# metagentools/VStrains

Measured on AMD Instinct MI355X. Metric: PE read pairs/sec through PE-link inference (GFA index + packed reads in HBM -> node_mat/short_mat), higher is better.
Workload: dtype u32

## Files before the change

### vstrains_amd/csrc/vs_api.hip

```cpp
#include <stdarg.h>
#include <stdio.h>
#include <stdlib.h>
#include <string.h>

#include "vs_internal.h"

static thread_local std::string g_create_err;

int vs_fail(vs_ctx *ctx, int code, const char *fmt, ...) {
    char buf[512];
    va_list ap;
    va_start(ap, fmt);
    vsnprintf(buf, sizeof buf, fmt, ap);
    va_end(ap);
    if (ctx) ctx->err = buf; else g_create_err = buf;
    return code;
}

static bool env_on(const char *name) {
    const char *v = getenv(name);
    return v && atoi(v) != 0;
}

void vs_tuning_load(VsTuning &t, bool experiment) {
    t = VsTuning();
    if (!experiment) return;
    if (const char *v = getenv("VS_EPT")) t.ept = (uint32_t)atoi(v) & ~1u;
    if (const char *v = getenv("VS_GRID_PER_CU")) t.grid_per_cu = atoi(v) > 0 ? (uint32_t)atoi(v) : 128u;
    if (const char *v = getenv("VS_ACC_FILL")) t.acc_fill_pct = atoi(v);
    if (const char *v = getenv("VS_ACC_TASKS")) t.acc_tasks = atoi(v) > 0 ? (uint32_t)atoi(v) : 0u;
    if (const char *v = getenv("VS_SHORTCUT")) t.shortcut = atoi(v) != 0 ? 1 : 0;
    if (const char *v = getenv("VS_ADAPT_GRID")) t.adapt_grid = atoi(v) != 0 ? 1 : 0;
    if (const char *v = getenv("VS_ACC_ROWS")) t.acc_rows = atoi(v) != 0 ? 1 : 0;
    if (const char *v = getenv("VS_LTAB_BITS")) t.ltab_bits = atoi(v) >= 0 && atoi(v) <= 31 ? atoi(v) : -1;
    if (const char *v = getenv("VS_ROWS_KEYS")) t.rows_keys = atoi(v) >= 2 && atoi(v) <= 65536 ? (uint32_t)atoi(v) : 0u;
    if (const char *v = getenv("VS_ROWS_SUB")) t.rows_sub = atoi(v) >= 1024 ? (uint32_t)atoi(v) : 0u;
    if (const char *v = getenv("VS_ROWS_PER_STRIP")) t.rows_per_strip = atoi(v) > 0 && atoi(v) <= 64 ? (uint32_t)atoi(v) : 0u;
    if (const char *v = getenv("VS_LOCUS_STAGE")) t.locus_stage = atoi(v) >= 0 ? atoi(v) : -1;
    t.no_sort = env_on("VS_NO_SORT");
    t.locus_global = env_on("VS_LOCUS_GLOBAL");
    t.no_fast = env_on("VS_NO_FAST");
    t.no_std = env_on("VS_NO_STD");
    t.no_agg = env_on("VS_NO_AGG");
    t.no_mid = env_on("VS_NO_MID");
}

extern "C" {

int vs_abi_version(void) { return VS_ABI_VERSION; }

int vs_device_count(void) {
    int n = 0;
    if (hipGetDeviceCount(&n) != hipSuccess) return 0;
    return n;
}

const char *vs_last_error(const vs_ctx *ctx) { return ctx ? ctx->err.c_str() : g_create_err.c_str(); }

int vs_ctx_create(int device, vs_ctx **out) {
    if (!out) return vs_fail(nullptr, VS_E_ARG, "vs_ctx_create: out is NULL");
    *out = nullptr;
    int n = 0;
    hipError_t e = hipGetDeviceCount(&n);
    if (e != hipSuccess || n <= 0)
        return vs_fail(nullptr, VS_E_HIP, "no HIP device available (%s); this library has no CPU path",
                       e == hipSuccess ? "device count 0" : hipGetErrorString(e));
    if (device < 0 || device >= n) return vs_fail(nullptr, VS_E_ARG, "device %d out of range (0..%d)", device, n - 1);
    e = hipSetDevice(device);
    if (e != hipSuccess) return vs_fail(nullptr, VS_E_HIP, "hipSetDevice(%d): %s", device, hipGetErrorString(e));
    vs_ctx *ctx = new vs_ctx();
    ctx->device = device;
    if (const char *ev = getenv("VS_EXPERIMENT")) ctx->experiment = strcmp(ev, "1") == 0;
    vs_tuning_load(ctx->tune, ctx->experiment);
    hipDeviceProp_t prop;
    if (hipGetDeviceProperties(&prop, device) == hipSuccess) ctx->n_cu = prop.multiProcessorCount;
    for (int i = 0; i < 5; i++) {
        e = hipEventCreate(&ctx->ev[i]);
        if (e != hipSuccess) {
            int rc = vs_fail(nullptr, VS_E_HIP, "hipEventCreate: %s", hipGetErrorString(e));
            delete ctx;
            return rc;
        }
    }
    *out = ctx;
    return VS_OK;
}

static void free_index(vs_ctx *ctx) {
    ctx->d_meta.reset();
    ctx->d_fwd.reset();
    ctx->d_table.reset();
    ctx->d_post.reset();
    ctx->d_slot_node.reset();
    ctx->has_index = false;
    ctx->index_bytes = 0;
}

void vs_ctx_free_index(vs_ctx *ctx) { free_index(ctx); }

void vs_ctx_destroy(vs_ctx *ctx) {
    if (!ctx) return;
    (void)hipSetDevice(ctx->device);
    (void)hipStreamSynchronize(ctx->stream);
    for (FqStage &st : ctx->fq_stage) {
        if (st.in_flight && st.done) (void)hipEventSynchronize(st.done);
        if (st.done) (void)hipEventDestroy(st.done);
    }
    for (int i = 0; i < 5; i++)
        if (ctx->ev[i]) (void)hipEventDestroy(ctx->ev[i]);
    delete ctx;
}

int vs_ctx_set_stream(vs_ctx *ctx, void *stream) {
    if (!ctx) return VS_E_ARG;
    ctx->stream = (hipStream_t)stream;
    return VS_OK;
}

int vs_ctx_keep_masks(vs_ctx *ctx, int on) {
    if (!ctx) return VS_E_ARG;
    ctx->keep_masks = on != 0;
// ... 170 lines not shown
```

### vstrains_amd/csrc/vs_pe.hip

```cpp
#include <stdio.h>
#include <stdlib.h>
#include <string.h>

#include <vector>

#include "vs_internal.h"
#include "vs_acc_tasks.h"
#include "vs_pe_pack.h"

#define TPB 256
#define LCAP 20u
__device__ __forceinline__ const uint32_t *vs_row_quad(const uint32_t *__restrict__ lists, const uint32_t *__restrict__ hi, uint64_t row, uint32_t q) {
    return q < LC / 4u ? lists + row * LC + 4u * q : hi + row * 4u;
}
#define EMPTY_NODE 0xFFFFFFFFu

struct PeParams {
    VsIndexDev idx;
    VsReadsDev rd;
    uint32_t *node_mat, *short_mat;
    unsigned long long *stats;
    uint32_t ept, pmax, words_cap, pool, pool_bits;
    uint64_t n_tiles;
    uint32_t *slow_list, *slow_count;
// ... 1502 lines not shown
                    const uint32_t ys[4] = {yv.x, yv.y, yv.z, yv.w};
                    uint32_t key[4], seen[4], at[4];
#pragma unroll
                    for (uint32_t j = 0; j < 4u; j++) {
                        key[j] = kbase + ys[j];
                        at[j] = RsTable::slot(key[j]);
                        seen[j] = s_key[at[j]];
                    }
#pragma unroll
                    for (uint32_t j = 0; j < 4u; j++) {
                        if (q4 + j >= n || (MODE && ys[j] < x)) continue;
                        if (seen[j] == key[j]) {
                            atomicAdd(&s_cnt[at[j]], wgt);
                        } else if (!vs_cell_claim<RsTable>(s_key, s_cnt, &s_used, key[j], at[j], wgt)) {
                            atomicAdd(&s_lost, 1u);
                            vs_mark_tile(tile_map, T, (uint32_t)MODE, x, ys[j]);
                            atomicAdd(mat + cell0 + (key[j] - align), wgt);
                        }
                    }
                };
                add_quad(yq, 4u * q);
                if (n > 16u && q == 0u) add_quad(*(const VsQuad *)(lists_hi + (uint64_t)(p0 & 0x07FFFFFFu) * 4u), 16u);
            }
            if ((pass & 3u) == 3u) {
                __syncthreads();
                const bool spill = s_used > fill_limit || s_lost > 4096u;
                __syncthreads();
                if (spill) write_out();
            }
        }
        __syncthreads();
        write_out();
    }
}

#define VS_LOCUS_MISS 0xFFFFFFFFu
__device__ __forceinline__ uint32_t vs_locus_probe(const VsIndexDev &idx, uint64_t key) {
    const uint32_t mask = (1u << idx.table_bits) - 1u;
    uint32_t sl = vs_slot_of(key, idx.table_bits);
    const uint4 *tab = (const uint4 *)idx.table;
    for (;;) {
        const uint4 raw = tab[sl];
        const uint32_t node = idx.slot_node[sl];
        const uint64_t k = (uint64_t)raw.x | ((uint64_t)raw.y << 32);
        if (k == VS_EMPTY_KEY) return VS_LOCUS_MISS;
        if ((k & ~VS_MULTI_BIT) == key) return node;
        sl = (sl + 1u) & mask;
    }
}

__device__ __forceinline__ uint32_t vs_locus_key(const VsIndexDev &idx, const VsReadsDev &rd, uint64_t p) {
    const uint32_t mf = rd.meta[2 * p], mr = rd.meta[2 * p + 1];
    const uint32_t N = idx.n_nodes, w = idx.w, s = idx.s, K = idx.K;
    if ((((mf | mr) >> 24) & VS_FLAG_N) || (mf & VS_LEN_MASK) < K || (mr & VS_FILTER_LEN_MASK) < K) return N + 1u;
    const uint32_t rlen = mf & VS_LEN_MASK;
    const uint64_t base = (uint64_t)rd.woff[2 * p] * 16u;
    const bool inv = (mf >> 24) & VS_FLAG_INVALID;
    for (uint32_t j = vs_seed_phase(rlen, w, s); j + w <= rlen; j += s) {
        if (inv && vs_seed_dirty(rd.mask, base + j, w)) continue;
        uint32_t sr;
        const uint64_t key = vs_seed_key(rd.words, base + j, w, &sr);
        const uint32_t node = vs_locus_probe(idx, key);
        if (node != VS_LOCUS_MISS) return node;
    }
    return N;
}

__device__ __forceinline__ uint32_t vs_locus_key_end(const VsIndexDev &idx, const VsReadsDev &rd, uint64_t e) {
    const uint32_t m = rd.meta[e];
    const uint32_t N = idx.n_nodes, w = idx.w, s = idx.s, rlen = m & VS_LEN_MASK;
    const uint64_t base = (uint64_t)rd.woff[e] * 16u;
    const bool inv = (m >> 24) & VS_FLAG_INVALID;
    for (uint32_t j = vs_seed_phase(rlen, w, s); j + w <= rlen; j += s) {
        if (inv && vs_seed_dirty(rd.mask, base + j, w)) continue;
        uint32_t sr;
        const uint64_t key = vs_seed_key(rd.words, base + j, w, &sr);
        const uint32_t node = vs_locus_probe(idx, key);
        if (node != VS_LOCUS_MISS) return node;
    }
    return N;
}

#define LOCUS_TPB 1024
__global__ void __launch_bounds__(LOCUS_TPB)
k_locus_count(VsIndexDev idx, VsReadsDev rd, uint64_t n_pairs, uint32_t chunk, uint32_t n_wg, uint32_t *__restrict__ keys,
              uint32_t *__restrict__ cnt, uint32_t key_lo, uint32_t nk, uint32_t compute) {
    for (uint32_t i = threadIdx.x; i < nk; i += LOCUS_TPB) vs_lds[i] = 0;
    __syncthreads();
    const uint64_t lo = (uint64_t)blockIdx.x * chunk;
    const uint64_t hi = lo + chunk < n_pairs ? lo + chunk : n_pairs;
    for (uint64_t p = lo + threadIdx.x; p < hi; p += LOCUS_TPB) {
        uint32_t key;
        if (compute) {
            key = vs_locus_key(idx, rd, p);
            keys[p] = key;
        } else {
            key = keys[p];
        }
        if (key - key_lo < nk) atomicAdd(&vs_lds[key - key_lo], 1u);
    }
    __syncthreads();
    for (uint32_t i = threadIdx.x; i < nk; i += LOCUS_TPB) cnt[(uint64_t)(key_lo + i) * n_wg + blockIdx.x] = vs_lds[i];
}

struct LocusHdr {
    uint32_t mf, mr, ws, we, w0;
    bool live;
};
typedef uint32_t LocusQuad __attribute__((ext_vector_type(4)));
struct LocusQuads {
    LocusQuad q0, q1, q2, q3, q4;
};
struct LocusProbe {
    uint32_t res, j, sl, node, rlen, lbase;
    uint64_t key, gbase;
    uint4 raw;
    bool have, active, inv;
};
__global__ void __launch_bounds__(LOCUS_TPB)
k_locus_count_staged(VsIndexDev idx, VsReadsDev rd, uint64_t n_pairs, uint32_t chunk, uint32_t n_wg, uint32_t *__restrict__ keys,
                     uint32_t *__restrict__ cnt, uint32_t nk, uint32_t cap) {
    static_assert(LOCUS_STAGE_PAIRS == 64u && LOCUS_TPB / 64u == LOCUS_STAGE_WAVES, "a batch holds one pair per lane of a wavefront");
    const uint32_t tid = threadIdx.x, lane = tid & 63u, wv = tid >> 6;
    const uint32_t hist_words = (nk + 3u) & ~3u, buf_words = vs_locus_buf_words(cap);
    uint32_t *s_hist = vs_lds;
    uint32_t *s_buf = vs_lds + hist_words + wv * 2u * buf_words;
    for (uint32_t i = tid; i < nk; i += LOCUS_TPB) s_hist[i] = 0;
    __syncthreads();
    const uint64_t c_lo = (uint64_t)blockIdx.x * chunk, c_hi = c_lo + chunk < n_pairs ? c_lo + chunk : n_pairs;
    const uint32_t sub = (chunk + LOCUS_STAGE_WAVES - 1u) / LOCUS_STAGE_WAVES;
    const uint64_t hi = c_lo + (uint64_t)(wv + 1u) * sub < c_hi ? c_lo + (uint64_t)(wv + 1u) * sub : c_hi;
    const uint64_t lo = c_lo + (uint64_t)wv * sub < hi ? c_lo + (uint64_t)wv * sub : hi;
    const bool any = lo < hi;
    const uint32_t N = idx.n_nodes, w = idx.w, s = idx.s, K = idx.K, tmask = (1u << idx.table_bits) - 1u;
    const uint4 *tab = (const uint4 *)idx.table;

    auto load_hdr = [&](uint64_t P) -> LocusHdr {
        LocusHdr h = {0u, 0u, 0u, 0u, 0u, false};
        if (!any) return h;
        const uint64_t Pc = P < hi ? P : hi - 1u, q = P + lane < hi ? P + lane : hi - 1u;
        const uint2 m = *(const uint2 *)(rd.meta + 2u * q);
        h.mf = m.x;
        h.mr = m.y;
        h.ws = rd.woff[2u * q];
        h.we = rd.woff[2u * q + 2u];
        h.w0 = rd.woff[2u * Pc];
        h.live = P + lane < hi;
        return h;
    };
    auto cut = [&](const LocusHdr &h, uint32_t &w_end) -> uint32_t {
        const uint64_t m = __ballot(vs_locus_in_batch(h.live, h.w0, h.we, cap));
        const uint32_t n = (uint32_t)__popcll(m);
        w_end = n ? (uint32_t)__shfl((int)h.we, (int)(n - 1u)) : 0u;
        return n;
    };
#define LOCUS_EACH_QUAD(X) X(0) X(1) X(2) X(3) X(4)
    static_assert(LOCUS_STAGE_QUADS == 5u, "LOCUS_EACH_QUAD names the quads");
    auto stage_load = [&](bool on, uint32_t w_first, uint32_t w_end, LocusQuads &r) {
        LocusSpan sp = vs_locus_span(on ? w_first : 0u, on ? w_end : 0u);
        if (sp.quads > buf_words / 4u) sp.quads = buf_words / 4u;
        const LocusQuad *src = (const LocusQuad *)(rd.words + sp.first);
#define LOCUS_LOAD(k) r.q##k = src[lane + k * 64u < sp.quads ? lane + k * 64u : sp.quads - 1u];
        LOCUS_EACH_QUAD(LOCUS_LOAD)
#undef LOCUS_LOAD
    };
    auto stage_store = [&](bool on, uint32_t w_first, uint32_t w_end, const LocusQuads &r, uint32_t *buf) {
// ... 24 lines not shown
            return;
        }
        if (k == VS_EMPTY_KEY) {
            q.j += s;
            q.active = seek(q);
        } else {
            q.sl = (q.sl + 1u) & tmask;
        }
        if (q.active) {
            q.raw = tab[q.sl];
            q.node = idx.slot_node[q.sl];
        }
    };
    auto finish = [&](const LocusProbe &q, uint64_t p_first) {
        if (q.have) {
            keys[p_first + lane] = q.res;
            if (q.res < nk) atomicAdd(&s_hist[q.res], 1u);
        }
    };

    LocusQuads r;
    uint64_t pc = lo, po = lo;
    LocusHdr hc = load_hdr(pc);
    uint32_t wec, wen;
    uint32_t nc = cut(hc, wec);
    bool stc = nc != 0u;
    if (!nc && pc < hi) nc = 1u;
    stage_load(stc, hc.w0, wec, r);
    stage_store(stc, hc.w0, wec, r, s_buf);
    uint64_t pn = pc + nc;
    LocusHdr hn = load_hdr(pn);
    uint32_t nn = cut(hn, wen);
    bool stn = nn != 0u;
    if (!nn && pn < hi) nn = 1u;
    LocusProbe qo = {};
    for (uint32_t it = 0; pc < hi; it++) {
        LocusProbe qc = {};
        qc.have = lane < nc;
        qc.res = N + 1u;
        qc.rlen = hc.mf & VS_LEN_MASK;
        qc.inv = (hc.mf >> 24) & VS_FLAG_INVALID;
        qc.lbase = ((it & 1u) * buf_words + hc.ws - (hc.w0 & ~3u)) * 16u;
        qc.gbase = (uint64_t)hc.ws * 16u;
        if (qc.have && !stc) {
            qc.res = vs_locus_key(idx, rd, pc);
        } else if (qc.have && !((((hc.mf | hc.mr) >> 24) & VS_FLAG_N) || qc.rlen < K || (hc.mr & VS_FILTER_LEN_MASK) < K)) {
            qc.res = N;
            qc.j = vs_seed_phase(qc.rlen, w, s);
            qc.active = seek(qc);
        }
        if (!qc.active) qc.sl = 0;
        qc.raw = tab[qc.sl];
        qc.node = idx.slot_node[qc.sl];
        stage_load(stn, hn.w0, wen, r);
        const uint64_t p2 = pn + nn;
        const LocusHdr h2 = load_hdr(p2);
        look(qo);
        look(qc);
        while (qo.active) {
            look(qo);
            look(qc);
        }
        finish(qo, po);
        stage_store(stn, hn.w0, wen, r, s_buf + ((it + 1u) & 1u) * buf_words);
        uint32_t we2;
        uint32_t n2 = cut(h2, we2);
        const bool st2 = n2 != 0u;
        if (!n2 && p2 < hi) n2 = 1u;
        qo.res = qc.res; qo.j = qc.j; qo.sl = qc.sl; qo.node = qc.node; qo.rlen = qc.rlen; qo.lbase = qc.lbase; qo.key = qc.key;
        qo.gbase = qc.gbase; qo.raw = qc.raw; qo.have = qc.have; qo.active = qc.active; qo.inv = qc.inv;
        po = pc;
        pc = pn; hc = hn; nc = nn; stc = stn; wec = wen;
        pn = p2; hn = h2; nn = n2; stn = st2; wen = we2;
    }
    while (qo.active) look(qo);
    finish(qo, po);
    __syncthreads();
    for (uint32_t i = tid; i < nk; i += LOCUS_TPB) cnt[(uint64_t)i * n_wg + blockIdx.x] = s_hist[i];
}

__global__ void __launch_bounds__(LOCUS_TPB)
k_locus_scatter(uint32_t key_lo, uint32_t nk, uint64_t n_pairs, uint32_t chunk, uint32_t n_wg, const uint32_t *__restrict__ keys,
                const uint32_t *__restrict__ first, uint32_t *__restrict__ perm) {
    for (uint32_t i = threadIdx.x; i < nk; i += LOCUS_TPB) vs_lds[i] = first[(uint64_t)(key_lo + i) * n_wg + blockIdx.x];
    __syncthreads();
    const uint64_t lo = (uint64_t)blockIdx.x * chunk;
    const uint64_t hi = lo + chunk < n_pairs ? lo + chunk : n_pairs;
    for (uint64_t p = lo + threadIdx.x; p < hi; p += LOCUS_TPB) {
        const uint32_t key = keys[p];
        if (key - key_lo < nk) perm[atomicAdd(&vs_lds[key - key_lo], 1u)] = (uint32_t)p;
    }
}

__global__ void __launch_bounds__(TPB)
k_pe_locus(VsIndexDev idx, VsReadsDev rd, uint64_t n_pairs, uint32_t *__restrict__ keys, uint32_t *__restrict__ hist) {
    const uint64_t p = (uint64_t)blockIdx.x * TPB + threadIdx.x;
    if (p >= n_pairs) return;
    const uint32_t key = vs_locus_key(idx, rd, p);
    keys[p] = key;
    atomicAdd(&hist[key], 1u);
}

__global__ void __launch_bounds__(TPB)
k_pe_permute(uint64_t n_pairs, const uint32_t *__restrict__ keys, uint32_t *__restrict__ cursor, uint32_t *__restrict__ perm) {
    const uint64_t p = (uint64_t)blockIdx.x * TPB + threadIdx.x;
    if (p >= n_pairs) return;
    perm[atomicAdd(&cursor[keys[p]], 1u)] = (uint32_t)p;
}

#define MID_SLOTS 256u
#define MID_LIST 64u
#define MID_WORDS (4u * MID_SLOTS + 3u * 64u + 65u + 2u * MID_LIST + 4u)
__global__ void __launch_bounds__(TPB)
k_pe_mid(PeParams P, const uint32_t *__restrict__ in_list, const uint32_t *__restrict__ in_count, uint32_t in_cap,
         uint32_t *__restrict__ out_list, uint32_t *__restrict__ out_count) {
    __shared__ uint32_t s_all[(TPB / 64u) * MID_WORDS];
    const uint32_t lane = threadIdx.x & 63u, wv = threadIdx.x >> 6;
    uint32_t *s_key = s_all + wv * MID_WORDS, *s_cnt = s_key + MID_SLOTS, *s_minp = s_cnt + MID_SLOTS, *s_minj = s_minp + MID_SLOTS;
    uint32_t *s_pa = s_minj + MID_SLOTS, *s_pb = s_pa + 64u, *s_pc = s_pb + 64u, *s_pref = s_pc + 64u;
    uint32_t *s_lst = s_pref + 65u;
    uint32_t *s_flag = s_lst + 2u * MID_LIST;
    const uint32_t N = P.idx.n_nodes, w = P.idx.w, s = P.idx.s, K = P.idx.K, wv_seed = VS_SEED_VERIFIED(P.idx.w);
    uint32_t n_in = *in_count;
    if (n_in > in_cap) n_in = in_cap;
    const uint32_t n_waves = gridDim.x * (TPB / 64u);
    for (uint32_t li = blockIdx.x * (TPB / 64u) + wv; li < n_in; li += n_waves) {
        const uint32_t pair = in_list[li];
        if (lane < 4u) s_flag[lane] = 0u;
        vs_wave_sync();
        for (uint32_t side = 0; side < 2u; side++) {
            const uint64_t e = 2ull * pair + side;
            const uint32_t meta = P.rd.meta[e];
            const uint32_t rlen = meta & VS_LEN_MASK;
            const uint64_t rbase = (uint64_t)P.rd.woff[e] * 16u;
            const uint32_t *mk = ((meta >> 24) & VS_FLAG_INVALID) ? P.rd.mask : nullptr;
            const uint32_t nprobe = vs_seed_probes(rlen, w, s), phase = vs_seed_phase(rlen, w, s);
            for (uint32_t i = lane; i < MID_SLOTS; i += 64u) { s_key[i] = EMPTY_NODE; s_cnt[i] = 0u; s_minp[i] = 0xFFFFFFFFu; s_minj[i] = 0xFFFFFFFFu; }
            if (nprobe > 64u) { if (lane == 0u) s_flag[0] = 1u; }
            uint32_t c = 0u, pa = 0u, pb = 0u;
            if (lane < nprobe && nprobe <= 64u) {
                const uint32_t j = phase + lane * s;
                if (!(mk && vs_seed_dirty(mk, rbase + j, w))) {
                    uint32_t sr;
                    const uint64_t key = vs_seed_key(P.rd.words, rbase + j, w, &sr);
                    c = vs_probe(P.idx, key, sr, &pa, &pb);
                }
            }
            uint32_t incl = c;
#pragma unroll
            for (int d = 1; d < 64; d <<= 1) {
                const uint32_t t2 = __shfl_up(incl, d, 64);
                if (lane >= (uint32_t)d) incl += t2;
            }
            s_pa[lane] = pa; s_pb[lane] = pb; s_pc[lane] = c;
            s_pref[lane + 1u] = incl;
            if (lane == 0u) s_pref[0] = 0u;
            vs_wave_sync();
            const uint32_t total = s_pref[64];
            for (uint32_t t = lane; t < total; t += 64u) {
                const uint32_t pr = vs_upper_idx(s_pref, 65u, t);
                const uint32_t k2 = t - s_pref[pr], j = phase + pr * s;
                uint32_t node, pos, opp;
                VsNodeMeta nm;
                if (s_pc[pr] == 1u) {
                    node = s_pa[pr]; pos = s_pb[pr] & 0x7FFFFFFFu; opp = s_pb[pr] >> 31;
                    nm = P.idx.meta[node];
                } else {
                    const VsPosting po = vs_posting_unpack(P.idx.postings[s_pa[pr] + k2]);
                    node = po.node; pos = po.pos; opp = po.strand ^ (s_pb[pr] >> 31);
                    nm.woff = po.woff; nm.len = po.len;
                }
                const uint32_t q = opp ? nm.len - pos - w : pos;
                uint32_t a, qa, len;
// ... 382 lines not shown
    VS_HIP(ctx, ctx->d_dense.reserve(pl.dense_bytes, pl.dense_bytes, &dense_new));
    if (dense_new) {
        ctx->dense_nodes = idx.n_nodes;
        uint64_t N = idx.n_nodes ? idx.n_nodes : 1;
        VS_HIP(ctx, hipMemsetAsync(ctx->d_dense.ptr(), 0xFF, pl.dense_bytes, st));
        hipLaunchKernelGGL(k_dense_zero_cnt, dim3((unsigned)((N * pl.slow_grid + TPB - 1) / TPB)), dim3(TPB), 0, st,
                           ctx->d_dense.as<uint32_t>(), N, (uint64_t)pl.slow_grid);
    }
    VS_HIP(ctx, hipMemsetAsync(ctx->d_slow_count.ptr(), 0, sizeof(uint32_t) * vs_ctx::SC_WORDS, st));
    if (pl.use_sort) {
        VS_HIP(ctx, ctx->d_locus_keys.reserve(sizeof(uint32_t) * n_pairs));
        VS_HIP(ctx, ctx->d_perm.reserve(sizeof(uint32_t) * n_pairs));
        VS_HIP(ctx, ctx->d_locus_hist.reserve(sizeof(uint32_t) * pl.locus_hist_words));
        VS_HIP(ctx, ctx->d_scan_tmp.reserve(sizeof(uint64_t) * (pl.locus_hist_words / 2048 + 4)));
    }
    if (d_node_mat) {
        VS_HIP(ctx, ctx->d_lists.reserve(sizeof(uint32_t) * pl.list_words));
        VS_HIP(ctx, ctx->d_list_counts.reserve(sizeof(uint32_t) * (pl.list_ends + 2)));
    }

    PeParams P;
    P.idx = idx;
    P.rd = reads->dev();
    P.out_lists = ctx->d_lists.as<uint32_t>();
    P.out_counts = ctx->d_list_counts.as<uint32_t>();
    P.node_mat = d_node_mat;
    P.short_mat = d_short_mat;
    P.stats = (unsigned long long *)d_stats;
    P.ept = pl.ept;
    P.pmax = pl.pmax;
    P.words_cap = pl.words_cap;
    P.pool = pl.pool;
    P.pool_bits = pl.pool_bits;
    P.n_pairs = n_pairs;
    P.n_tiles = pl.n_tiles;
    P.tiles_per_wg = pl.tiles_per_wg;
    P.wpe = pl.wpe;
    P.magic_pmax = pl.magic_pmax;
    P.magic_wpe = pl.magic_wpe;
    P.perm = pl.use_sort ? ctx->d_perm.as<const uint32_t>() : nullptr;
    P.slow_list = ctx->d_slow_list.as<uint32_t>();
    P.slow_count = ctx->d_slow_count.as<uint32_t>();
    P.dbg_lists = d_dbg_lists;
    P.dbg_counts = d_dbg_counts;
    P.dbg_cap = dbg_cap;
    P.accumulate = d_node_mat ? 1u : 0u;
    P.out_rows = pl.use_rows;
    P.out_lists_hi = ctx->d_lists.as<uint32_t>() + pl.list_ends * LC;
    P.tile_map = d_node_mat ? d_tile_map : nullptr;
    P.tile_T = (idx.n_nodes + 63u) >> 6;
    P.shortcut = pl.shortcut;
    P.mid_fast = pl.mid_fast;

    const size_t lds = pl.lds_bytes;
    if (lds > 64u * 1024u)
        VS_HIP(ctx, hipFuncSetAttribute(tf->fn, hipFuncAttributeMaxDynamicSharedMemorySize, (int)lds));
    VS_HIP(ctx, hipEventRecord(ctx->ev[3], st));
    ctx->last_order_pairs = n_pairs;
    if (pl.use_sort) {
        const uint64_t nk = pl.locus_keys;
        ctx->last_launched |= pl.lds_sort ? VS_RAN_LOCUS_LDS_SORT : VS_RAN_LOCUS_GLOBAL_SORT;
        if (pl.lds_sort) {
            const uint32_t n_wg = LOCUS_WGS, chunk = pl.locus_chunk, per_pass = pl.locus_per_pass;
            const size_t lds_keys = sizeof(uint32_t) * per_pass;
            if (lds_keys > 64u * 1024u) {
                VS_HIP(ctx, hipFuncSetAttribute((const void *)k_locus_count, hipFuncAttributeMaxDynamicSharedMemorySize, (int)lds_keys));
                VS_HIP(ctx, hipFuncSetAttribute((const void *)k_locus_scatter, hipFuncAttributeMaxDynamicSharedMemorySize, (int)lds_keys));
            }
            if (pl.locus_stage_words && ((uintptr_t)reads->d_words & 15u) == 0u) {
                VS_HIP(ctx, hipFuncSetAttribute((const void *)k_locus_count_staged, hipFuncAttributeMaxDynamicSharedMemorySize, (int)pl.locus_lds_bytes));
                hipLaunchKernelGGL(k_locus_count_staged, dim3(n_wg), dim3(LOCUS_TPB), pl.locus_lds_bytes, st, idx, reads->dev(), n_pairs, chunk, n_wg,
                                   ctx->d_locus_keys.as<uint32_t>(), ctx->d_locus_hist.as<uint32_t>(), (uint32_t)nk, pl.locus_stage_words);
                ctx->last_launched |= VS_RAN_LOCUS_STAGED;
            } else {
                for (uint32_t key_lo = 0; key_lo < nk; key_lo += per_pass) {
                    const uint32_t n_here = (uint32_t)(nk - key_lo < per_pass ? nk - key_lo : per_pass);
                    hipLaunchKernelGGL(k_locus_count, dim3(n_wg), dim3(LOCUS_TPB), lds_keys, st, idx, reads->dev(), n_pairs, chunk, n_wg,
                                       ctx->d_locus_keys.as<uint32_t>(), ctx->d_locus_hist.as<uint32_t>(), key_lo, n_here, key_lo == 0u ? 1u : 0u);
                }
            }
            int rc = vs_scan_u32(ctx, ctx->d_locus_hist.as<const uint32_t>(), ctx->d_locus_hist.as<uint32_t>(), nk * n_wg,
                                 ctx->d_scan_tmp.as<uint64_t>(), nullptr);
            if (rc) return rc;
            for (uint32_t key_lo = 0; key_lo < nk; key_lo += per_pass) {
                const uint32_t n_here = (uint32_t)(nk - key_lo < per_pass ? nk - key_lo : per_pass);
                hipLaunchKernelGGL(k_locus_scatter, dim3(n_wg), dim3(LOCUS_TPB), lds_keys, st, key_lo, n_here, n_pairs, chunk, n_wg,
                                   ctx->d_locus_keys.as<const uint32_t>(), ctx->d_locus_hist.as<const uint32_t>(), ctx->d_perm.as<uint32_t>());
            }
        } else {
            VS_HIP(ctx, hipMemsetAsync(ctx->d_locus_hist.ptr(), 0, sizeof(uint32_t) * nk, st));
            const unsigned pg = (unsigned)((n_pairs + TPB - 1) / TPB);
            hipLaunchKernelGGL(k_pe_locus, dim3(pg), dim3(TPB), 0, st, idx, reads->dev(), n_pairs, ctx->d_locus_keys.as<uint32_t>(),
                               ctx->d_locus_hist.as<uint32_t>());
            int rc = vs_scan_u32(ctx, ctx->d_locus_hist.as<const uint32_t>(), ctx->d_locus_hist.as<uint32_t>(), nk,
                                 ctx->d_scan_tmp.as<uint64_t>(), nullptr);
            if (rc) return rc;
            hipLaunchKernelGGL(k_pe_permute, dim3(pg), dim3(TPB), 0, st, n_pairs, ctx->d_locus_keys.as<const uint32_t>(),
                               ctx->d_locus_hist.as<uint32_t>(), ctx->d_perm.as<uint32_t>());
        }
    }
    VS_HIP(ctx, hipEventRecord(ctx->ev[0], st));
    if (!d_node_mat) VS_HIP(ctx, hipEventRecord(ctx->ev[4], st));
    ctx->last_kernel = tf->name;
    {
        void *kargs[] = {(void *)&P};
        VS_HIP(ctx, hipLaunchKernel(tf->fn, dim3((unsigned)pl.grid), dim3(TTPB), kargs, lds, st));
    }
    if (d_node_mat) {
        const StdTable tab = pl.sw ? vs_std_table((int)pl.mode, true, pl.ad != 0u) : StdTable{pl.pool, 0u};
        ctx->last_handoff.pairs = n_pairs;
        ctx->last_handoff.list_ends = pl.list_ends;
        ctx->last_handoff.ept = pl.ept;
        ctx->last_handoff.rows = pl.use_rows;
        ctx->last_handoff.pool = tab.pool;
        ctx->last_handoff.trim = tab.trim;
        const int rc = pe_count_from_lists(ctx, pl, idx.n_nodes, 2ull * n_pairs, d_node_mat, d_short_mat, d_tile_map);
        if (rc) return rc;
    }
    VS_HIP(ctx, hipEventRecord(ctx->ev[1], st));
    const bool no_mid = ctx->tune.no_mid;
    ctx->last_launched |= no_mid ? 0u : VS_RAN_PE_MID;
    if (!no_mid) {
        hipLaunchKernelGGL(k_pe_mid, dim3((unsigned)ctx->n_cu * 8u), dim3(TPB), 0, st, P, ctx->d_slow_list.as<const uint32_t>(),
                           ctx->d_slow_count.as<const uint32_t>(), (uint32_t)n_pairs, ctx->d_slow_list2.as<uint32_t>(), ctx->d_slow_count.as<uint32_t>() + vs_ctx::SC_SLOW);
        hipLaunchKernelGGL(k_pe_slow, dim3(pl.slow_grid), dim3(TPB), 0, st, P, ctx->d_dense.as<uint32_t>(), (uint32_t)n_pairs,
                           ctx->d_slow_list2.as<const uint32_t>(), ctx->d_slow_count.as<const uint32_t>() + vs_ctx::SC_SLOW);
    } else {
        hipLaunchKernelGGL(k_pe_slow, dim3(pl.slow_grid), dim3(TPB), 0, st, P, ctx->d_dense.as<uint32_t>(), (uint32_t)n_pairs,
                           ctx->d_slow_list.as<const uint32_t>(), ctx->d_slow_count.as<const uint32_t>());
    }
    ctx->last_overflow.pairs = n_pairs;
    ctx->last_overflow.no_mid = no_mid ? 1u : 0u;
    VS_HIP(ctx, hipEventRecord(ctx->ev[2], st));
    VS_HIP(ctx, hipGetLastError());
    return VS_OK;
}

extern "C" int vs_pe_count(vs_ctx *ctx, const vs_reads *reads, uint32_t *d_node_mat, uint32_t *d_short_mat, uint64_t *d_stats) {
    if (!ctx || !reads || !d_node_mat || !d_short_mat || !d_stats) return VS_E_ARG;
    return pe_launch(ctx, reads, d_node_mat, d_short_mat, d_stats, nullptr, nullptr, 0);
}

extern "C" int vs_pe_count_tracked(vs_ctx *ctx, const vs_reads *reads, uint32_t *d_node_mat, uint32_t *d_short_mat, uint64_t *d_stats,
                                   uint8_t *d_tile_map) {
    if (!ctx || !reads || !d_node_mat || !d_short_mat || !d_stats || !d_tile_map) return VS_E_ARG;
    return pe_launch(ctx, reads, d_node_mat, d_short_mat, d_stats, nullptr, nullptr, 0, d_tile_map);
}

extern "C" int vs_counts_zero_tracked(vs_ctx *ctx, uint32_t *d_node_mat, uint32_t *d_short_mat, uint32_t n, uint8_t *d_tile_map) {
    if (!ctx || (n && (!d_node_mat || !d_short_mat || !d_tile_map))) return vs_fail(ctx, VS_E_ARG, "vs_counts_zero_tracked: bad argument");
    if (!n) return VS_OK;
    VS_HIP(ctx, hipSetDevice(ctx->device));
    const uint32_t T = (n + 63u) >> 6;
    const uint64_t tiles = 2ull * T * T;
    if (tiles > 0x7FFFFFFFull) return vs_fail(ctx, VS_E_RANGE, "vs_counts_zero_tracked: %u nodes make more tiles than one launch takes", n);
    hipLaunchKernelGGL(k_zero_tiles, dim3((unsigned)((tiles + 63u) / 64u)), dim3(64), 0, ctx->stream, d_node_mat, d_short_mat, n, T, d_tile_map, tiles);
    VS_HIP(ctx, hipGetLastError());
    return VS_OK;
}

static PePlan pe_lists_plan(vs_ctx *ctx, uint32_t n_nodes, uint64_t n_ends, bool tile_map) {
    if (ctx->experiment) vs_tuning_load(ctx->tune, true);
    PePlanIn in;
    in.n_nodes = n_nodes; in.K = STD_K; in.w = STD_W; in.s = STD_S;
    in.n_cu = (uint32_t)ctx->n_cu;
    in.n_ends = n_ends; in.max_len = 150u;
    in.count = true; in.tile_map = tile_map;
    in.tune = ctx->tune;
// ... 303 lines not shown
```

### vstrains_amd/csrc/vs_pe_plan.h

```cpp
#ifndef VS_PE_PLAN_H
#define VS_PE_PLAN_H
#include <stddef.h>
#include <stdint.h>
#include <stdio.h>

#include <initializer_list>

#include "../../include/vstrains_hip.h"

#if defined(__HIPCC__)
#define VS_PLAN_FN __host__ __device__ inline
#else
#define VS_PLAN_FN inline
#endif

struct VsTuning {
    uint32_t ept = 0;
    uint32_t grid_per_cu = 128;
    int acc_fill_pct = -1;
    uint32_t acc_tasks = 0;
    int shortcut = -1;
    int adapt_grid = -1;
    int acc_rows = -1;
    int ltab_bits = -1;
    uint32_t rows_keys = 0, rows_sub = 0;
    uint32_t rows_per_strip = 0;
    bool no_sort = false, locus_global = false, no_fast = false, no_std = false, no_agg = false;
    bool no_mid = false;
    int locus_stage = -1;
};

VS_PLAN_FN uint32_t vs_seed_phase(uint32_t len, uint32_t w, uint32_t s) {
    return len < w ? 0u : ((len - w) % s + s) / 2u;
}
VS_PLAN_FN uint32_t vs_seed_probes(uint32_t len, uint32_t w, uint32_t s) {
    if (len < w) return 0u;
    return (len - w + 1u) / s;
}
#define VS_SEED_VERIFIED(w) ((w) <= 31u ? (w) : 0u)

#define LC 16u
#define PPT 2u
#define TTPB 256
#define PPT_LONG 1u
#define CHUNK (TTPB * PPT)
#define ACC_TPB 1024
#define ACC_BITS 14
#define ACC_SLOTS (1u << ACC_BITS)
#define ACC_PPW 64u
#define ACC_TASK_WORDS 480u
#define ACC_TASK_CAP (2u * ACC_TASK_WORDS)
#define ACC_TASK_MIN 40u
#define ACC_QUEUE 64u
#define ACC_TASK_PLAN_CAP (ACC_TASK_CAP - 2u * ACC_QUEUE)
#define ACC_BINS 24u
#define ROWS_KEYS 65536u
#define ROWS_SUB ((1u << 26) - 1024u)
#define RS_BITS 13
#define RS_SLOTS (1u << RS_BITS)
#define LOCUS_LDS_KEYS 36864u
#define LOCUS_LDS_MAX_PASSES 4u
#define LOCUS_WGS 256u
#define LOCUS_STAGE_WAVES 16u
#define LOCUS_STAGE_PAIRS 64u
#define LOCUS_STAGE_QUADS 5u
#define LOCUS_STAGE_SLACK 16u
#define LOCUS_STAGE_MAX (LOCUS_STAGE_QUADS * 4u * LOCUS_STAGE_PAIRS - LOCUS_STAGE_SLACK)
#define LOCUS_STAGE_MIN_PAIRS 48u
#define LOCUS_LDS_WORDS 40960u
#define SLOW_WORDS_PER_NODE 6u
#define LDS_BUDGET_BYTES (64u * 1024u)
#define NI_CAP 4096u

VS_PLAN_FN bool vs_locus_in_batch(bool exists, uint32_t w_first, uint32_t w_pair_end, uint32_t cap) {
    return exists && w_pair_end - w_first <= cap;
}
struct LocusBatch {
    uint32_t n;
    uint32_t staged;
};
VS_PLAN_FN LocusBatch vs_locus_batch(const uint32_t *woff, uint64_t p0, uint64_t hi, uint32_t cap) {
    LocusBatch b = {0u, 1u};
    if (p0 >= hi) return b;
    const uint32_t w_first = woff[2u * p0];
    while (b.n < LOCUS_STAGE_PAIRS && vs_locus_in_batch(p0 + b.n < hi, w_first, p0 + b.n < hi ? woff[2u * (p0 + b.n) + 2u] : 0u, cap)) b.n++;
    if (!b.n) { b.n = 1u; b.staged = 0u; }
    return b;
}
struct LocusSpan {
    uint32_t first, quads;
};
VS_PLAN_FN LocusSpan vs_locus_span(uint32_t w_first, uint32_t w_end) {
    LocusSpan sp;
    sp.first = w_first & ~3u;
    sp.quads = (w_end + 4u - sp.first + 3u) / 4u;
    return sp;
}
VS_PLAN_FN uint32_t vs_locus_buf_words(uint32_t cap) { return ((cap + 3u) & ~3u) + LOCUS_STAGE_SLACK; }

struct TileLayout {
    uint32_t woff, gend, meta, inv, words, pcnt, pa, pb, hkey, hcnt, hminp, hminj, ns, state, list, owner, misc, total;
};
VS_PLAN_FN TileLayout tile_layout(uint32_t ept, uint32_t pmax, uint32_t words_cap, uint32_t pool, uint32_t list_trim = 0u) {
    TileLayout t;
    uint32_t o = 0;
    const uint32_t NI = ept * pmax;
    t.woff = o;  o += 2u * ((ept + 2u) & ~1u);
    t.gend = o;  o += 2u * ept;
    t.meta = o;  o += 2u * ept;
    t.inv = o;   o += ept;
    t.words = o; o += 2u * (words_cap + 8u);
    t.pcnt = o;  o += NI + 1u;
    t.pa = o;    o += NI;
    t.pb = o;    o += NI;
    t.hkey = o;  o += pool;
    t.hcnt = o;  o += pool;
    t.hminp = o; o += pool;
    t.hminj = o; o += pool;
    t.ns = o;    o += ept;
    t.state = o; o += ept;
    t.list = o;
    t.owner = o; o += (ept * LC - list_trim > CHUNK ? ept * LC - list_trim : CHUNK);
    t.misc = o;  o += 16u;
    t.total = o;
    return t;
}

#define STD_EPT (TTPB / 4u)
#define STD_POOL_BITS 10u
#define STD_K 56u
#define STD_W 31u
#define STD_S 26u
#define STD2_EPT 60u
#define STD2_POOL_BITS 10u
#define STD2_K 128u
#define STD2_W 63u
#define STD2_S 66u
struct StdShape {
    uint32_t mode, sw, sp;
};
constexpr StdShape VS_STD_SHAPES[] = {{1u, 10u, 4u}, {1u, 8u, 3u}, {1u, 7u, 2u}, {1u, 7u, 3u}, {2u, 16u, 2u}};
struct StdTable {
    uint32_t pool, trim;
};
VS_PLAN_FN constexpr StdTable vs_std_table(int mode, bool std_shape, bool ad) {
    return std_shape && !ad ? StdTable{768u, mode == 2 ? 192u : 64u} : StdTable{1u << (mode == 2 ? STD2_POOL_BITS : STD_POOL_BITS), 0u};
}

inline uint32_t slow_grid_for(uint32_t n_nodes) {
    const uint64_t per_wg = sizeof(uint32_t) * (uint64_t)SLOW_WORDS_PER_NODE * (n_nodes ? n_nodes : 1u);
    uint64_t g = (4ull << 30) / per_wg;
    return (uint32_t)(g < 64u ? 64u : g > 2048u ? 2048u : g);
}

inline uint32_t pool_for(uint32_t ept, uint32_t *bits) {
    uint32_t b = 6;
    while ((1u << b) < 16u * ept) b++;
    *bits = b;
    return 1u << b;
}

inline size_t lds_bytes(uint32_t ept, uint32_t pmax, uint32_t words_cap) {
    uint32_t bits;
    uint32_t pool = pool_for(ept, &bits);
    return (size_t)tile_layout(ept, pmax, words_cap, pool).total * sizeof(uint32_t);
}

struct PePlanIn {
    uint32_t n_nodes = 0, K = 0, w = 0, s = 0;
    uint64_t n_seed_pos = 0, n_distinct = 0;
    uint32_t max_node_len = 0, n_cu = 0;
    uint64_t n_ends = 0;
    uint32_t max_len = 0;
    bool has_mask = false, has_inv4 = false;
    bool count = false, tile_map = false;
    VsTuning tune;
};

struct PePlan {
    int status;
    char msg[128];
    uint32_t ept, pmax, wpe, pool, pool_bits, words_cap, magic_pmax, magic_wpe;
    uint64_t lds_bytes;
    uint32_t mode, sw, sp, ad;
    uint64_t n_tiles, grid, list_ends, list_words;
    uint32_t tiles_per_wg, shortcut, mid_fast;
    uint32_t use_sort, lds_sort, locus_chunk, locus_per_pass;
    uint64_t locus_keys, locus_hist_words;
    uint32_t locus_stage_words;
    uint64_t locus_lds_bytes;
    uint32_t use_rows, use_table, mark_tiles;
    uint32_t acc_grid, acc_per_wg, acc_fill, acc_task_cap;
    uint64_t rows_sub_pairs;
    uint32_t rows_ltab_bits, rows_keys, rows_fill, rows_per_strip;
    uint32_t slow_grid;
    uint64_t dense_bytes;
};

inline PePlan vs_pe_plan(const PePlanIn &in) {
    PePlan p = {};
    const VsTuning &tn = in.tune;
    const uint64_t n_pairs = in.n_ends / 2;
    if (n_pairs == 0) return p;
    const uint32_t maxlen = in.max_len, N = in.n_nodes;
    if (N > 0x01FFFFFEu) {
        p.status = VS_E_RANGE;
        snprintf(p.msg, sizeof p.msg, "more than 2^25-2 nodes");
        return p;
    }
    const uint32_t wpe = maxlen ? (maxlen + 15u) / 16u : 1u;
    uint32_t pmax = vs_seed_probes(maxlen, in.w, in.s);
    if (!pmax) pmax = 1u;
    uint32_t ept = tn.ept ? tn.ept : STD_EPT;
    if (ept < 2 || ept > TTPB / 2u) ept = STD_EPT;
    while (ept > 2 && (ept * pmax > NI_CAP || lds_bytes(ept, pmax, ept * wpe) > LDS_BUDGET_BYTES)) ept -= 2;
    if (!tn.ept) {
        for (size_t fit : {(size_t)32000, (size_t)40000}) {
            uint32_t e2 = ept;
            while (e2 > STD_EPT / 2u && lds_bytes(e2, pmax, e2 * wpe) > fit) e2 -= 2;
            if (lds_bytes(e2, pmax, e2 * wpe) <= fit) { ept = e2; break; }
        }
    }
    size_t lds = lds_bytes(ept, pmax, ept * wpe);
    if (lds > 160u * 1024u) {
        p.status = VS_E_RANGE;
        snprintf(p.msg, sizeof p.msg, "reads of %u bases with k+1=%u need %zu B of LDS per pair (limit 160 KiB)", maxlen, in.K, lds);
        return p;
    }
    p.ept = ept;
    p.pmax = pmax;
    p.wpe = wpe;
    p.words_cap = ept * wpe;
    p.pool = pool_for(ept, &p.pool_bits);
    p.magic_pmax = pmax > 1u ? (uint32_t)(0x100000000ull / pmax) + 1u : 0u;
    p.magic_wpe = wpe > 1u ? (uint32_t)(0x100000000ull / wpe) + 1u : 0u;
    p.slow_grid = slow_grid_for(N);
    p.dense_bytes = sizeof(uint32_t) * (uint64_t)SLOW_WORDS_PER_NODE * (N ? N : 1) * p.slow_grid;

    p.use_sort = !tn.no_sort && n_pairs >= 4096 && n_pairs < 0xFFFFFFF0ull;
    if (p.use_sort) {
        const uint64_t nk = (uint64_t)N + 2u;
        const bool fits_lds = nk <= LOCUS_LDS_MAX_PASSES * LOCUS_LDS_KEYS;
        p.locus_keys = nk;
        p.locus_hist_words = fits_lds ? nk * LOCUS_WGS : nk;
        p.lds_sort = fits_lds && !tn.locus_global;
        if (p.lds_sort) {
            p.locus_chunk = (uint32_t)((n_pairs + LOCUS_WGS - 1) / LOCUS_WGS);
            p.locus_per_pass = (uint32_t)(nk < LOCUS_LDS_KEYS ? nk : LOCUS_LDS_KEYS);
            p.locus_lds_bytes = sizeof(uint32_t) * (uint64_t)p.locus_per_pass;
            if (nk < LOCUS_LDS_KEYS && tn.locus_stage != 0) {
                const uint32_t hist = ((uint32_t)nk + 3u) & ~3u;
                uint32_t room = ((LOCUS_LDS_WORDS - hist) / (2u * LOCUS_STAGE_WAVES) - LOCUS_STAGE_SLACK) & ~3u;
                if (room > LOCUS_STAGE_MAX) room = LOCUS_STAGE_MAX;
                uint32_t cap = room / (2u * wpe) >= LOCUS_STAGE_MIN_PAIRS ? room : 0u;
                if (tn.locus_stage > 0) cap = (uint32_t)tn.locus_stage < room ? (uint32_t)tn.locus_stage : room;
                if (cap) {
                    p.locus_stage_words = cap;
                    p.locus_lds_bytes = sizeof(uint32_t) * (uint64_t)(hist + 2u * LOCUS_STAGE_WAVES * vs_locus_buf_words(cap));
                }
            }
        }
    }

    p.use_table = tn.no_agg ? 0u : 1u;
    const bool fits32 = 2ull * N * N < 0xFFFFFFFFull;
    bool use_rows = tn.acc_rows >= 0 ? tn.acc_rows != 0 : !fits32;
    if (N == 0 || !p.use_table) use_rows = false;
    if (!use_rows && !fits32) p.use_table = 0u;
    p.use_rows = use_rows;
    p.n_tiles = (n_pairs + ept / 2 - 1) / (ept / 2);
    p.list_ends = p.n_tiles * ept;
    p.list_words = p.list_ends * (use_rows ? LC + 4u : LC) + 16u;

    p.shortcut = in.n_distinct && in.n_seed_pos < 2 * in.n_distinct ? 1u : 0u;
    if (tn.shortcut >= 0) p.shortcut = (uint32_t)tn.shortcut;
    if (VS_SEED_VERIFIED(in.w) == 0u) p.shortcut = 0u;

    const bool straight = (!in.has_mask || in.has_inv4) && in.max_node_len < (1u << 23) && !tn.no_fast;
    const bool fast = straight && in.s <= 32u && maxlen <= 128u + in.w + 32u;
    p.mid_fast = fast && VS_SEED_VERIFIED(in.w) ? 1u : 0u;
    uint32_t long_reach = 0;
    for (uint32_t len = in.K; len <= maxlen; len++) {
        const uint32_t behind = len - vs_seed_phase(len, in.w, in.s) - VS_SEED_VERIFIED(in.w);
        long_reach = behind > long_reach ? behind : long_reach;
    }
    const bool fast_long = !fast && straight && in.s <= 128u && long_reach <= 256u && maxlen < 512u;
    p.mode = fast ? 1u : fast_long ? 2u : 0u;
    const bool shape1 = p.mode == 1u && ept == STD_EPT && p.pool_bits == STD_POOL_BITS && maxlen <= 159u && in.K == STD_K && in.w == STD_W && in.s == STD_S;
    const bool shape2 = p.mode == 2u && ept == STD2_EPT && p.pool_bits == STD2_POOL_BITS && in.K == STD2_K && in.w == STD2_W && in.s == STD2_S;
    if (in.count && !tn.no_std && (shape1 || shape2))
        for (const StdShape &sh : VS_STD_SHAPES)
            if (sh.mode == p.mode && sh.sw == wpe && sh.sp == pmax) { p.sw = wpe; p.sp = pmax; }
    if (p.sw) {
        p.ad = tn.adapt_grid >= 0 ? tn.adapt_grid != 0 : in.n_distinct && in.n_seed_pos >= 6u * in.n_distinct;
        const StdTable tab = vs_std_table((int)p.mode, true, p.ad);
        lds = (size_t)tile_layout(ept, pmax, ept * wpe, tab.pool, tab.trim).total * sizeof(uint32_t);
    }
    p.lds_bytes = lds;
    const uint64_t max_grid = (uint64_t)in.n_cu * tn.grid_per_cu;
    p.grid = p.n_tiles < max_grid ? p.n_tiles : max_grid;
    p.tiles_per_wg = (uint32_t)((p.n_tiles + p.grid - 1) / p.grid);
    p.grid = (p.n_tiles + p.tiles_per_wg - 1) / p.tiles_per_wg;
    if (!in.count) return p;

    const uint64_t slots_pairs = p.list_ends / 2;
    if (!use_rows) {
        p.mark_tiles = in.tile_map;
        p.acc_grid = in.n_cu * 32u;
        p.acc_per_wg = (uint32_t)((slots_pairs + p.acc_grid - 1) / p.acc_grid);
        p.acc_per_wg = (p.acc_per_wg + ACC_TPB - 1) / ACC_TPB * ACC_TPB;
        p.acc_grid = (uint32_t)((slots_pairs + p.acc_per_wg - 1) / p.acc_per_wg);
        if (p.acc_grid > in.n_cu * 2u) p.acc_grid = in.n_cu * 2u;
        p.acc_fill = ACC_SLOTS / 16u;
        if (tn.acc_fill_pct >= 0) p.acc_fill = (uint32_t)((uint64_t)ACC_SLOTS * (uint32_t)tn.acc_fill_pct / 100u);
        p.acc_task_cap = tn.acc_tasks >= ACC_TASK_MIN && tn.acc_tasks < ACC_TASK_PLAN_CAP ? tn.acc_tasks : ACC_TASK_PLAN_CAP;
        return p;
    }
    const uint64_t sub_max = tn.rows_sub ? (uint64_t)tn.rows_sub : (uint64_t)ROWS_SUB;
    p.rows_sub_pairs = slots_pairs < sub_max ? slots_pairs : sub_max;
    p.rows_ltab_bits = 10;
    while ((1ull << p.rows_ltab_bits) < 2u * p.rows_sub_pairs && p.rows_ltab_bits < 31u) p.rows_ltab_bits++;
    if (tn.ltab_bits >= 0) p.rows_ltab_bits = (uint32_t)tn.ltab_bits;
    const uint32_t keys_max = tn.rows_keys ? tn.rows_keys : ROWS_KEYS;
    p.rows_keys = N < keys_max ? N : keys_max;
    p.rows_fill = RS_SLOTS / 2u;
    if (tn.acc_fill_pct >= 0) p.rows_fill = (uint32_t)((uint64_t)RS_SLOTS * (uint32_t)tn.acc_fill_pct / 100u);
    if (p.rows_fill > RS_SLOTS - 1024u) p.rows_fill = RS_SLOTS - 1024u;
    p.rows_per_strip = tn.rows_per_strip ? tn.rows_per_strip : 2u;
    return p;
}

#endif
// ... 1 lines not shown
```

Baseline: 1.528 billion.

## Restructure locus scatter with batched key prefetch, block remap and key-range splitting

The locus scatter kernel now loads eight keys per thread ahead of use (double-buffered), issues the LDS atomics in a batch, and then writes perm. This is meant to hide global load latency. Block indices are remapped so neighbouring workgroups take chunks spread across the array. For large inputs the scatter is split into up to four launches over key sub-ranges, so each pass writes to a narrower perm region and gets better write locality. The cost is re-reading the keys array once per launch, plus extra registers per thread.

```diff
diff --git a/vstrains_amd/csrc/vs_api.hip b/vstrains_amd/csrc/vs_api.hip
--- a/vstrains_amd/csrc/vs_api.hip
+++ b/vstrains_amd/csrc/vs_api.hip
@@ -37,6 +37,7 @@
     if (const char *v = getenv("VS_ROWS_SUB")) t.rows_sub = atoi(v) >= 1024 ? (uint32_t)atoi(v) : 0u;
     if (const char *v = getenv("VS_ROWS_PER_STRIP")) t.rows_per_strip = atoi(v) > 0 && atoi(v) <= 64 ? (uint32_t)atoi(v) : 0u;
     if (const char *v = getenv("VS_LOCUS_STAGE")) t.locus_stage = atoi(v) >= 0 ? atoi(v) : -1;
+    if (const char *v = getenv("VS_LOCUS_SCATTER")) t.locus_scatter = atoi(v) > 0 ? atoi(v) : 0;
     t.no_sort = env_on("VS_NO_SORT");
     t.locus_global = env_on("VS_LOCUS_GLOBAL");
     t.no_fast = env_on("VS_NO_FAST");
diff --git a/vstrains_amd/csrc/vs_pe.hip b/vstrains_amd/csrc/vs_pe.hip
--- a/vstrains_amd/csrc/vs_pe.hip
+++ b/vstrains_amd/csrc/vs_pe.hip
@@ -1608,6 +1608,7 @@
 }
 
 #define LOCUS_TPB 1024
+#define LOCUS_SCATTER_U 8u
 __global__ void __launch_bounds__(LOCUS_TPB)
 k_locus_count(VsIndexDev idx, VsReadsDev rd, uint64_t n_pairs, uint32_t chunk, uint32_t n_wg, uint32_t *__restrict__ keys,
               uint32_t *__restrict__ cnt, uint32_t key_lo, uint32_t nk, uint32_t compute) {
@@ -1798,13 +1799,38 @@
 __global__ void __launch_bounds__(LOCUS_TPB)
 k_locus_scatter(uint32_t key_lo, uint32_t nk, uint64_t n_pairs, uint32_t chunk, uint32_t n_wg, const uint32_t *__restrict__ keys,
                 const uint32_t *__restrict__ first, uint32_t *__restrict__ perm) {
-    for (uint32_t i = threadIdx.x; i < nk; i += LOCUS_TPB) vs_lds[i] = first[(uint64_t)(key_lo + i) * n_wg + blockIdx.x];
+    uint32_t wg = blockIdx.x;
+    if ((n_wg & 7u) == 0u) wg = (blockIdx.x & 7u) * (n_wg >> 3) + (blockIdx.x >> 3);
+    for (uint32_t i = threadIdx.x; i < nk; i += LOCUS_TPB) vs_lds[i] = first[(uint64_t)(key_lo + i) * n_wg + wg];
     __syncthreads();
-    const uint64_t lo = (uint64_t)blockIdx.x * chunk;
+    const uint64_t lo = (uint64_t)wg * chunk;
     const uint64_t hi = lo + chunk < n_pairs ? lo + chunk : n_pairs;
-    for (uint64_t p = lo + threadIdx.x; p < hi; p += LOCUS_TPB) {
-        const uint32_t key = keys[p];
-        if (key - key_lo < nk) perm[atomicAdd(&vs_lds[key - key_lo], 1u)] = (uint32_t)p;
+    if (lo >= hi || !nk) return;
+    const uint32_t span = (uint32_t)(hi - lo), turns = (span + LOCUS_SCATTER_U * LOCUS_TPB - 1u) / (LOCUS_SCATTER_U * LOCUS_TPB);
+    const uint32_t idle = (threadIdx.x & 63u) < nk ? threadIdx.x & 63u : 0u;
+    uint32_t k[LOCUS_SCATTER_U], kn[LOCUS_SCATTER_U], at[LOCUS_SCATTER_U];
+    bool on[LOCUS_SCATTER_U];
+    auto request = [&](uint32_t q0, uint32_t *dst) {
+#pragma unroll
+        for (uint32_t j = 0; j < LOCUS_SCATTER_U; j++) {
+            const uint32_t q = q0 + j * LOCUS_TPB;
+            dst[j] = keys[lo + (q < span ? q : span - 1u)];
+        }
+    };
+    uint32_t q0 = threadIdx.x;
+    request(q0, kn);
+    for (uint32_t t = 0; t < turns; t++, q0 += LOCUS_SCATTER_U * LOCUS_TPB) {
+#pragma unroll
+        for (uint32_t j = 0; j < LOCUS_SCATTER_U; j++) k[j] = kn[j];
+        request(q0 + LOCUS_SCATTER_U * LOCUS_TPB, kn);
+#pragma unroll
+        for (uint32_t j = 0; j < LOCUS_SCATTER_U; j++) {
+            on[j] = q0 + j * LOCUS_TPB < span && k[j] - key_lo < nk;
+            at[j] = atomicAdd(&vs_lds[on[j] ? k[j] - key_lo : idle], on[j] ? 1u : 0u);
+        }
+#pragma unroll
+        for (uint32_t j = 0; j < LOCUS_SCATTER_U; j++)
+            if (on[j]) perm[at[j]] = (uint32_t)(lo + q0 + j * LOCUS_TPB);
     }
 }
 
@@ -2353,8 +2379,9 @@
             int rc = vs_scan_u32(ctx, ctx->d_locus_hist.as<const uint32_t>(), ctx->d_locus_hist.as<uint32_t>(), nk * n_wg,
                                  ctx->d_scan_tmp.as<uint64_t>(), nullptr);
             if (rc) return rc;
-            for (uint32_t key_lo = 0; key_lo < nk; key_lo += per_pass) {
-                const uint32_t n_here = (uint32_t)(nk - key_lo < per_pass ? nk - key_lo : per_pass);
+            const uint32_t sc_keys = pl.locus_scatter_keys;
+            for (uint32_t key_lo = 0; key_lo < nk; key_lo += sc_keys) {
+                const uint32_t n_here = (uint32_t)(nk - key_lo < sc_keys ? nk - key_lo : sc_keys);
                 hipLaunchKernelGGL(k_locus_scatter, dim3(n_wg), dim3(LOCUS_TPB), lds_keys, st, key_lo, n_here, n_pairs, chunk, n_wg,
                                    ctx->d_locus_keys.as<const uint32_t>(), ctx->d_locus_hist.as<const uint32_t>(), ctx->d_perm.as<uint32_t>());
             }
diff --git a/vstrains_amd/csrc/vs_pe_plan.h b/vstrains_amd/csrc/vs_pe_plan.h
--- a/vstrains_amd/csrc/vs_pe_plan.h
+++ b/vstrains_amd/csrc/vs_pe_plan.h
@@ -28,6 +28,7 @@
     bool no_sort = false, locus_global = false, no_fast = false, no_std = false, no_agg = false;
     bool no_mid = false;
     int locus_stage = -1;
+    int locus_scatter = 0;
 };
 
 VS_PLAN_FN uint32_t vs_seed_phase(uint32_t len, uint32_t w, uint32_t s) {
@@ -68,6 +69,8 @@
 #define LOCUS_STAGE_MAX (LOCUS_STAGE_QUADS * 4u * LOCUS_STAGE_PAIRS - LOCUS_STAGE_SLACK)
 #define LOCUS_STAGE_MIN_PAIRS 48u
 #define LOCUS_LDS_WORDS 40960u
+#define LOCUS_SCATTER_PAIRS 2621440u
+#define LOCUS_SCATTER_MAX 4u
 #define SLOW_WORDS_PER_NODE 6u
 #define LDS_BUDGET_BYTES (64u * 1024u)
 #define NI_CAP 4096u
@@ -189,6 +192,7 @@
     uint64_t locus_keys, locus_hist_words;
     uint32_t locus_stage_words;
     uint64_t locus_lds_bytes;
+    uint32_t locus_scatter_keys;
     uint32_t use_rows, use_table, mark_tiles;
     uint32_t acc_grid, acc_per_wg, acc_fill, acc_task_cap;
     uint64_t rows_sub_pairs;
@@ -248,6 +252,11 @@
             p.locus_chunk = (uint32_t)((n_pairs + LOCUS_WGS - 1) / LOCUS_WGS);
             p.locus_per_pass = (uint32_t)(nk < LOCUS_LDS_KEYS ? nk : LOCUS_LDS_KEYS);
             p.locus_lds_bytes = sizeof(uint32_t) * (uint64_t)p.locus_per_pass;
+            const uint64_t sc_pairs = tn.locus_scatter > 0 ? (uint64_t)tn.locus_scatter : LOCUS_SCATTER_PAIRS;
+            uint64_t launches = (n_pairs + sc_pairs - 1u) / sc_pairs;
+            if (launches > LOCUS_SCATTER_MAX) launches = LOCUS_SCATTER_MAX;
+            const uint64_t sc_keys = (nk + launches - 1u) / launches;
+            p.locus_scatter_keys = sc_keys < p.locus_per_pass ? (uint32_t)sc_keys : p.locus_per_pass;
             if (nk < LOCUS_LDS_KEYS && tn.locus_stage != 0) {
                 const uint32_t hist = ((uint32_t)nk + 3u) & ~3u;
                 uint32_t room = ((LOCUS_LDS_WORDS - hist) / (2u * LOCUS_STAGE_WAVES) - LOCUS_STAGE_SLACK) & ~3u;
```

New measurement: 1.549 billion (median of 6 runs). +1.4%, better.
